# InterDigitalInc/VersatileFilmGrain

Hardware: NVIDIA B200
Metric: 4k_10bit_420_frames_per_sec_device_resident (higher is better)
Workload: dtype int32

## Files before the change

### versatilefilmgrain_b200/csrc/fgs_fast.h

```cpp
#pragma once
#include <stddef.h>
#include <type_traits>
#include "fgs_task.h"

namespace vfgs {

VFGS_HD uint32_t prmt(uint32_t a, uint32_t b, uint32_t sel)
{
#if defined(__CUDA_ARCH__)
	uint32_t d;
	asm("prmt.b32 %0, %1, %2, %3;" : "=r"(d) : "r"(a), "r"(b), "r"(sel));
	return d;
#else
	const uint64_t src = ((uint64_t)b << 32) | a;
	uint32_t d = 0;
	for (int i = 0; i < 4; i++) {
		const uint32_t n = (sel >> (4 * i)) & 0xf;
		uint32_t byte = (uint32_t)(src >> (8 * (n & 7))) & 0xff;
		if (n & 8) byte = (byte & 0x80) ? 0xff : 0x00;
		d |= byte << (8 * i);
	}
	return d;
#endif
}
// ... 651 lines not shown
	g[6] = blend<6>(g[6], u0, u1, w_cur, w_up); g[7] = blend<7>(g[7], u0, u1, w_cur, w_up);
}
template <bool IN16, bool OUT8, int NSH, bool MSB = false>
VFGS_HD void wide_line(const WideLane& L, int rc, int w_cur, int w_up, const WideUp& U, int ru,
                       const uint32_t* raw, uint32_t* outw)
{
	uint32_t a0, a1, b0, b1;
	octet(L.own0 + rc, a0, a1);
	octet(L.own1 + rc, b0, b1);
	int ga[8], gb[8];
	octet_to_ints(a0, a1, ga);
	octet_to_ints(b0, b1, gb);
	int hl = L.has_left ? lds_s8(L.lh + rc) : 0;
	int hr = L.has_right ? lds_s8(L.rh + rc) : 0;
	if (w_cur) {
		uint32_t u0, u1;
		octet(U.own0 + ru, u0, u1);
		blend_octet(ga, u0, u1, w_cur, w_up);
		octet(U.own1 + ru, u0, u1);
		blend_octet(gb, u0, u1, w_cur, w_up);
		if (L.has_left) hl = (hl * w_cur + lds_s8(U.lh + ru) * w_up + 16) >> 5;
		if (L.has_right) hr = (hr * w_cur + lds_s8(U.rh + ru) * w_up + 16) >> 5;
	}
	const int f0 = (hl + 3 * ga[0] + ga[1] + 2) >> 2;
	const int f15 = (gb[6] + 3 * gb[7] + hr + 2) >> 2;
	if (NSH == 3) {
		const int f7 = (ga[6] + 3 * ga[7] + gb[0] + 2) >> 2;
		const int f8 = (ga[7] + 3 * gb[0] + gb[1] + 2) >> 2;
		ga[7] = f7; gb[0] = f8;
	}
	ga[0] = L.has_left ? f0 : ga[0];
	gb[7] = L.has_right ? f15 : gb[7];
	if (IN16) {
		uint32_t cv[8];
		if (MSB) msb_to_lsb<8>(raw, cv);
		const uint32_t* r = MSB ? cv : raw;
		scale_add_clip_16bit<OUT8>(L.lut, L.lo2, L.hi2, ga, r, outw);
		scale_add_clip_16bit<OUT8>(L.lut, L.lo2, L.hi2, gb, r + 4, outw + (OUT8 ? 2 : 4));
	} else {
		scale_add_clip_8bit(L.lut, L.lo2, L.hi2, ga, raw[0], raw[1], outw[0], outw[1]);
		scale_add_clip_8bit(L.lut, L.lo2, L.hi2, gb, raw[2], raw[3], outw[2], outw[3]);
	}
}

#ifndef VFGS_WIDE16_LB
#define VFGS_WIDE16_LB 2
#endif
#ifndef VFGS_WIDE16_LBW
#define VFGS_WIDE16_LBW 4
#endif
#ifndef VFGS_WIDE16_LB8
#define VFGS_WIDE16_LB8 2
#endif
template <bool IN16, bool OUT8, int NSH, bool ALLWIDE = false, bool MSB = false>
VFGS_HD void wide_task_body(const FgsParams& p, smem_addr_t lut, const TaskGeom& t, int k0, int lane)
{
	const int c = t.c;
	const smem_addr_t img = lut + (smem_addr_t)(ptrdiff_t)p.fimg_off[c];
	const Plane& pl = p.comp[c];
	const int ysh = (c && p.suby > 1) ? 1 : 0;
	constexpr int n = 1 << NSH;
	constexpr int LB = !IN16 ? VFGS_FAST_LB16 : OUT8 ? VFGS_WIDE16_LB8 : ALLWIDE ? VFGS_WIDE16_LBW : VFGS_WIDE16_LB;
	static_assert(LB >= 2, "both vertical-overlap lines of a block-row must fall into the first group of lines");
	constexpr int IB = IN16 ? 2 : 1, OB = (IN16 && !OUT8) ? 2 : 1;
	constexpr int RW = IN16 ? 8 : 4, OW = OB == 2 ? 8 : 4;

	const int cl0 = (t.r * 16) >> ysh;
	int cl1 = cl0 + (16 >> ysh);
	if (cl1 > pl.lines) cl1 = pl.lines;
	const int nl = cl1 - cl0;
	if (nl <= 0) return;

	const long long in_pitch = pl.in_row_bytes, out_pitch = pl.out_row_bytes;
	const uint8_t* src = pl.in + (long long)t.f * p.in_frame_bytes + (long long)cl0 * in_pitch + (long long)k0 * IB;
	uint8_t* dst = pl.out + (long long)t.f * p.out_frame_bytes + (long long)cl0 * out_pitch + (long long)k0 * OB;

	uint32_t raw[LB][RW];
#pragma unroll
	for (int q = 0; q < LB; q++) {
		if (IN16) ld_global_32(src + (q < nl ? q : nl - 1) * in_pitch, raw[q]);
		else ld_global_16(src + (q < nl ? q : nl - 1) * in_pitch, raw[q]);
	}

	const int b0 = k0 >> NSH, b1 = (k0 + 15) >> NSH;
	WideLane L;
	L.has_left = b0 > 0;
	L.has_right = b1 + 1 < p.nb;
	L.stride = p.fpat_stride[c];
	L.lut = lut + (smem_addr_t)(c * kLutBytes + lane * 4);
	constexpr int kOutBias = (IN16 && OUT8) ? 2 : 0;
	L.lo2 = (uint32_t)(p.lo[c] + kOutBias) * 0x00010001u; L.hi2 = (uint32_t)(p.hi[c] + kOutBias) * 0x00010001u;

	const int srow = t.r - p.stream_row0;
	const uint16_t* w_cur = p.woffs + (((long long)t.f * p.stream_rows + srow) * p.spitch + 1 + b0) * 4 + c;
	auto windows = [&](const uint16_t* w, smem_addr_t& own0, smem_addr_t& own1, smem_addr_t& lh, smem_addr_t& rh) {
		own0 = img + (smem_addr_t)w[0];
		own1 = NSH == 4 ? own0 + 8 : img + (smem_addr_t)w[4];
		lh = rh = own0;
		if (L.has_left) lh = img + (smem_addr_t)(w[-4] + n - 1);
		if (L.has_right) rh = img + (smem_addr_t)w[NSH == 4 ? 4 : 8];
	};
	windows(w_cur, L.own0, L.own1, L.lh, L.rh);
	WideUp U;
	U.own0 = U.own1 = U.lh = U.rh = L.own0;
	bool ovl = t.r > 0;
	if (ovl) windows(w_cur - p.spitch * 4, U.own0, U.own1, U.lh, U.rh);

	int rc = 0;
	const uint8_t* nxt = src + LB * in_pitch;
#pragma unroll 1
	for (int base = 0; base < nl; base += LB) {
#pragma unroll
		for (int q = 0; q < LB; q++) {
			const int line = base + q;
			uint32_t w[OW];
			int wc = 0, wu = 0, ru = 0;
			if (q == 0 && ovl) { wc = ysh ? 20 : 12; wu = ysh ? 20 : 24; ru = (16 >> ysh) * L.stride; }
			if (q == 1 && ovl && !ysh) { wc = 24; wu = 12; ru = 17 * L.stride; }
			wide_line<IN16, OUT8, NSH, MSB>(L, rc, wc, wu, U, ru, raw[q], w);
			if (MSB && OB == 2) lsb_to_msb<OW>(w);
			if (IN16) ld_global_32_if(nxt, raw[q], line + LB < nl);
			else ld_global_16_if(nxt, raw[q], line + LB < nl);
			if (line < nl) {
				if (OB == 2) st_global_32(dst, w);
				else st_global_16(dst, w);
			}
			rc += L.stride; nxt += in_pitch; dst += out_pitch;
		}
		ovl = false;
	}
}

template <bool OUT8>
VFGS_HD void scale_add_clip_uv_16bit(smem_addr_t lut_u, smem_addr_t lut_v, uint32_t lo2, uint32_t hi2, const int* gu, const int* gv,
                                     const uint32_t raw[4], uint32_t* outw)
{
	constexpr int kRound = OUT8 ? 0x28000 : 0x8000;
	uint32_t r[4];
#pragma unroll
	for (int k = 0; k < 4; k++) {
		const int s_lo = (int)lds32(lut_u | (smem_addr_t)((raw[k] << 5) & 0x7f80u));
		const int s_hi = (int)lds32(lut_v | (smem_addr_t)(shr_fma<11>(raw[k]) & 0x7f80u));
		const int a_lo = s_lo * gu[k] + kRound;
		const int a_hi = s_hi * gv[k] + kRound;
		const uint32_t d2 = prmt((uint32_t)a_lo, (uint32_t)a_hi, 0x7632);
		const uint32_t v2 = min_u16x2(raw[k], 0x3fff3fffu);
		r[k] = min_s16x2(add_max_s16x2(v2, d2, lo2), hi2);
	}
	if (OUT8) {
#pragma unroll
		for (int k = 0; k < 4; k++) r[k] *= 64u;
		outw[0] = prmt(r[0], r[1], 0x7531);
		outw[1] = prmt(r[2], r[3], 0x7531);
	} else {
		outw[0] = r[0]; outw[1] = r[1]; outw[2] = r[2]; outw[3] = r[3];
	}
}
VFGS_HD void scale_add_clip_uv_8bit(smem_addr_t lut_u, smem_addr_t lut_v, uint32_t lo2, uint32_t hi2, const int* gu, const int* gv,
                                    uint32_t raw0, uint32_t raw1, uint32_t& out0, uint32_t& out1)
{
	uint32_t r[4];
#pragma unroll
	for (int k = 0; k < 4; k++) {
		const uint32_t v2 = prmt(k < 2 ? raw0 : raw1, 0u, (k & 1) ? 0x4342 : 0x4140);
		const int s_lo = (int)lds32(lut_u | (smem_addr_t)((v2 << 7) & 0x7f80u));
		const int s_hi = (int)lds32(lut_v | (smem_addr_t)(shr_fma<9>(v2) & 0x7f80u));
		const int a_lo = s_lo * gu[k] + 0x8000;
		const int a_hi = s_hi * gv[k] + 0x8000;
		const uint32_t d2 = prmt((uint32_t)a_lo, (uint32_t)a_hi, 0x7632);
		r[k] = min_s16x2(add_max_s16x2(v2, d2, lo2), hi2);
	}
	out0 = prmt(r[0], r[1], 0x6420);
	out1 = prmt(r[2], r[3], 0x6420);
}

struct UvLane {
	smem_addr_t own_u, own_v;
	smem_addr_t lh_u, rh_u, lh_v, rh_v;
	smem_addr_t lut_u, lut_v;
	int stride;
	bool has_left, has_right;
	uint32_t lo2, hi2;
};
struct UvUp {
	smem_addr_t own_u, own_v, lh_u, rh_u, lh_v, rh_v;
};

VFGS_HD void block_octet(smem_addr_t own, smem_addr_t lh, smem_addr_t rh, smem_addr_t up_own, smem_addr_t up_lh, smem_addr_t up_rh,
                         bool has_left, bool has_right, int rc, int w_cur, int w_up, int ru, int g[8])
{
	uint32_t a0, a1;
	octet(own + rc, a0, a1);
	octet_to_ints(a0, a1, g);
	int hl = has_left ? lds_s8(lh + rc) : 0;
	int hr = has_right ? lds_s8(rh + rc) : 0;
	if (w_cur) {
		uint32_t u0, u1;
		octet(up_own + ru, u0, u1);
		blend_octet(g, u0, u1, w_cur, w_up);
		if (has_left) hl = (hl * w_cur + lds_s8(up_lh + ru) * w_up + 16) >> 5;
		if (has_right) hr = (hr * w_cur + lds_s8(up_rh + ru) * w_up + 16) >> 5;
	}
	const int f0 = (hl + 3 * g[0] + g[1] + 2) >> 2;
	const int f7 = (g[6] + 3 * g[7] + hr + 2) >> 2;
	g[0] = has_left ? f0 : g[0];
	g[7] = has_right ? f7 : g[7];
}

template <bool IN16, bool OUT8>
VFGS_HD void uv_line(const UvLane& L, int rc, int w_cur, int w_up, const UvUp& U, int ru, const uint32_t* raw, uint32_t* outw)
{
	int gu[8], gv[8];
	block_octet(L.own_u, L.lh_u, L.rh_u, U.own_u, U.lh_u, U.rh_u, L.has_left, L.has_right, rc, w_cur, w_up, ru, gu);
	block_octet(L.own_v, L.lh_v, L.rh_v, U.own_v, U.lh_v, U.rh_v, L.has_left, L.has_right, rc, w_cur, w_up, ru, gv);
	if (IN16) {
		uint32_t cv[8];
		msb_to_lsb<8>(raw, cv);
		scale_add_clip_uv_16bit<OUT8>(L.lut_u, L.lut_v, L.lo2, L.hi2, gu, gv, cv, outw);
		scale_add_clip_uv_16bit<OUT8>(L.lut_u, L.lut_v, L.lo2, L.hi2, gu + 4, gv + 4, cv + 4, outw + (OUT8 ? 2 : 4));
	} else {
		scale_add_clip_uv_8bit(L.lut_u, L.lut_v, L.lo2, L.hi2, gu, gv, raw[0], raw[1], outw[0], outw[1]);
		scale_add_clip_uv_8bit(L.lut_u, L.lut_v, L.lo2, L.hi2, gu + 4, gv + 4, raw[2], raw[3], outw[2], outw[3]);
	}
}

template <bool IN16, bool OUT8, bool ALLWIDE = false>
VFGS_HD void uv_task_body(const FgsParams& p, smem_addr_t lut, const TaskGeom& t, int k0, int lane)
{
	const Plane& pl = p.comp[1];
	const int ysh = p.suby > 1 ? 1 : 0;
	constexpr int LB = !IN16 ? VFGS_FAST_LB16 : OUT8 ? VFGS_WIDE16_LB8 : ALLWIDE ? VFGS_WIDE16_LBW : VFGS_WIDE16_LB;
	static_assert(LB >= 2, "both vertical-overlap lines of a block-row must fall into the first group of lines");
	constexpr int IB = IN16 ? 2 : 1, OB = (IN16 && !OUT8) ? 2 : 1;
	constexpr int RW = IN16 ? 8 : 4, OW = OB == 2 ? 8 : 4;

	const int cl0 = (t.r * 16) >> ysh;
	int cl1 = cl0 + (16 >> ysh);
	if (cl1 > pl.lines) cl1 = pl.lines;
	const int nl = cl1 - cl0;
	if (nl <= 0) return;

	const long long in_pitch = pl.in_row_bytes, out_pitch = pl.out_row_bytes;
	const uint8_t* src = pl.in + (long long)t.f * p.in_frame_bytes + (long long)cl0 * in_pitch + (long long)k0 * 2 * IB;
	uint8_t* dst = pl.out + (long long)t.f * p.out_frame_bytes + (long long)cl0 * out_pitch + (long long)k0 * 2 * OB;

	uint32_t raw[LB][RW];
#pragma unroll
	for (int q = 0; q < LB; q++) {
		if (IN16) ld_global_32(src + (q < nl ? q : nl - 1) * in_pitch, raw[q]);
		else ld_global_16(src + (q < nl ? q : nl - 1) * in_pitch, raw[q]);
	}

	const int b = k0 >> 3;
	UvLane L;
	L.has_left = b > 0;
	L.has_right = b + 1 < p.nb;
	L.stride = p.fpat_stride[1];
	L.lut_u = lut + (smem_addr_t)(kLutBytes + lane * 4);
	L.lut_v = lut + (smem_addr_t)(2 * kLutBytes + lane * 4);
	constexpr int kOutBias = (IN16 && OUT8) ? 2 : 0;
	L.lo2 = (uint32_t)(p.lo[1] + kOutBias) * 0x00010001u; L.hi2 = (uint32_t)(p.hi[1] + kOutBias) * 0x00010001u;

	const smem_addr_t img_u = lut + (smem_addr_t)(ptrdiff_t)p.fimg_off[1], img_v = lut + (smem_addr_t)(ptrdiff_t)p.fimg_off[2];
	const int srow = t.r - p.stream_row0;
	const uint16_t* w_u = p.woffs + (((long long)t.f * p.stream_rows + srow) * p.spitch + 1 + b) * 4 + 1;
	auto windows = [&](const uint16_t* w, UvUp& o) {
		o.own_u = img_u + (smem_addr_t)w[0];
		o.own_v = img_v + (smem_addr_t)w[1];
		o.lh_u = o.rh_u = o.own_u; o.lh_v = o.rh_v = o.own_v;
		if (L.has_left) { o.lh_u = img_u + (smem_addr_t)(w[-4] + 7); o.lh_v = img_v + (smem_addr_t)(w[-3] + 7); }
		if (L.has_right) { o.rh_u = img_u + (smem_addr_t)w[4]; o.rh_v = img_v + (smem_addr_t)w[5]; }
	};
	UvUp C;
	windows(w_u, C);
	L.own_u = C.own_u; L.own_v = C.own_v; L.lh_u = C.lh_u; L.rh_u = C.rh_u; L.lh_v = C.lh_v; L.rh_v = C.rh_v;
	UvUp U = C;
	bool ovl = t.r > 0;
	if (ovl) windows(w_u - p.spitch * 4, U);

	int rc = 0;
	const uint8_t* nxt = src + LB * in_pitch;
#pragma unroll 1
	for (int base = 0; base < nl; base += LB) {
#pragma unroll
		for (int q = 0; q < LB; q++) {
			const int line = base + q;
			uint32_t w[OW];
			int wc = 0, wu = 0, ru = 0;
			if (q == 0 && ovl) { wc = ysh ? 20 : 12; wu = ysh ? 20 : 24; ru = (16 >> ysh) * L.stride; }
			if (q == 1 && ovl && !ysh) { wc = 24; wu = 12; ru = 17 * L.stride; }
			uv_line<IN16, OUT8>(L, rc, wc, wu, U, ru, raw[q], w);
			if (OB == 2) lsb_to_msb<OW>(w);
			if (IN16) ld_global_32_if(nxt, raw[q], line + LB < nl);
			else ld_global_16_if(nxt, raw[q], line + LB < nl);
			if (line < nl) {
				if (OB == 2) st_global_32(dst, w);
				else st_global_16(dst, w);
			}
			rc += L.stride; nxt += in_pitch; dst += out_pitch;
		}
		ovl = false;
	}
}

template <bool IN16, bool OUT8, bool EDGE = false, bool ALLWIDE = false, bool SEMI = false>
VFGS_HD void process_task_fast(const FgsParams& p, smem_addr_t lut, uint32_t task, int lane)
{
	TaskGeom t;
	t.f = (int)fastdiv(task, p.div_ftasks);
	uint32_t q = task - (uint32_t)t.f * (uint32_t)p.ftasks_per_frame;
	t.c = 0;
	if (q >= (uint32_t)p.ftasks[0]) { q -= (uint32_t)p.ftasks[0]; t.c = 1; }
	if (t.c == 1 && q >= (uint32_t)p.ftasks[1]) { q -= (uint32_t)p.ftasks[1]; t.c = 2; }
	const uint32_t unit = q * 32u + (uint32_t)lane;
	const uint32_t upr = (uint32_t)p.funits_per_row[t.c];
	if (unit >= upr * (uint32_t)p.rows) return;
	const uint32_t row = fastdiv(unit, p.div_funits[t.c]);
	t.r = p.row_begin + (int)row;
	t.seg = 0;
	static_assert(!(ALLWIDE && EDGE), "the EDGE variant has no wide path");
	static_assert(!(SEMI && EDGE), "the EDGE variant has no semi-planar form");
	if constexpr (SEMI) {
		const int u = (int)(unit - row * upr);
		if (t.c) uv_task_body<IN16, OUT8, ALLWIDE>(p, lut, t, u * 8, lane);
		else wide_task_body<IN16, OUT8, 4, ALLWIDE, IN16>(p, lut, t, u * 16, lane);
		return;
	}
	if (ALLWIDE || (!EDGE && p.fwide[t.c])) {
		const int k0 = (int)(unit - row * upr) * 16;
		if (t.c && p.subx > 1) wide_task_body<IN16, OUT8, 3, ALLWIDE>(p, lut, t, k0, lane);
		else wide_task_body<IN16, OUT8, 4, ALLWIDE>(p, lut, t, k0, lane);
		return;
	}
	if (ALLWIDE) return;
	const int k0 = (int)(unit - row * upr) * kSamplesPerLane;
	if (t.c && p.subx > 1) fast_task_body<IN16, OUT8, 3, EDGE>(p, lut, t, k0, lane);
	else fast_task_body<IN16, OUT8, 4, EDGE>(p, lut, t, k0, lane);
}

}
```

### versatilefilmgrain_b200/csrc/vfgs_b200.cu

```cuda
#include <cuda_runtime.h>
#include <stdarg.h>
#include <stdio.h>
#include <stdlib.h>
#include <string.h>
#include <time.h>
#include <algorithm>
#include <memory>
#include <mutex>
#include <thread>
#include <vector>

#include "../../include/vfgs_b200.h"
#include "../../include/vfgs_fw.h"
#include "../../include/vfgs_hw.h"
#include "../../include/yuv.h"
#include "vfgs_kernels.cuh"
#include "fw_host.h"

using namespace vfgs;

namespace {

struct Slot {
	uint8_t* d_in = nullptr;
// ... 293 lines not shown
}
int make_geometry(Geometry& g, int width, int height, int out_depth) { return make_geometry(g, hw(), width, height, out_depth); }

void fill_common(FgsParams& p, const Geometry& g, const StateRef& s)
{
	memset(&p, 0, sizeof(p));
	fill_state_params(p, *s.h, *s.bi);
	p.nb = g.nb; p.R = g.R;
	p.in_bytes = (int)g.in_sample; p.out_bytes = (int)g.out_sample;
	p.blob = s.img ? s.img->d_blob : nullptr;
	p.fblob = s.img ? s.img->d_fblob : nullptr;
	p.spitch = g.spitch;
}

typedef void (*GrainKernel)(const FgsParams);
enum KernelKind { kGeneral = 0, kFast = 1, kGather = 2, kFastEdge = 3 };

template <bool FOLD, bool SHIFT>
GrainKernel gather_kernel(const FgsParams& p)
{
	if (p.msb_in)
		return p.out_bytes == 1 ? fgs_apply_gather_kernel<true, true, FOLD, SHIFT, true> : fgs_apply_gather_kernel<true, false, FOLD, SHIFT, true>;
	return p.in_bytes == 1 ? fgs_apply_gather_kernel<false, false, FOLD, SHIFT>
	     : p.out_bytes == 1 ? fgs_apply_gather_kernel<true, true, FOLD, SHIFT> : fgs_apply_gather_kernel<true, false, FOLD, SHIFT>;
}
GrainKernel gather_kernel(const FgsParams& p, bool fold, bool shift)
{
	return fold ? (shift ? gather_kernel<true, true>(p) : gather_kernel<true, false>(p))
	            : (shift ? gather_kernel<false, true>(p) : gather_kernel<false, false>(p));
}

int launch_apply(const FgsParams& p, cudaStream_t stream, KernelKind kind = kGeneral, int gather_smem = 0, bool gather_fold = false,
                 bool gather_shift = false)
{
	Context& c = g_ctx;
	if (p.total_tasks <= 0) return VFGS_B200_OK;
	if (p.total_tasks >= (1ll << 31)) return set_err(VFGS_B200_ERR_ARG, "batch too large for one launch (%lld warp-tasks): split the call", p.total_tasks);
	GrainKernel kern = fgs_apply_kernel;
	int threads = kCtaThreads, smem = p.blob_bytes;
	if (kind == kFast || kind == kFastEdge) {
		const bool allwide = kind == kFast && p.in_bytes == 2 && p.out_bytes == 2 && p.fallwide;
		if (kind == kFast && p.ilv[1])
			kern = allwide ? fgs_apply_fast_kernel<true, false, false, true, true>
			     : p.in_bytes == 1 ? fgs_apply_fast_kernel<false, false, false, false, true>
			     : p.out_bytes == 1 ? fgs_apply_fast_kernel<true, true, false, false, true> : fgs_apply_fast_kernel<true, false, false, false, true>;
		else if (allwide)
			kern = fgs_apply_fast_kernel<true, false, false, true>;
		else if (kind == kFast)
			kern = p.in_bytes == 1 ? fgs_apply_fast_kernel<false, false>
			     : p.out_bytes == 1 ? fgs_apply_fast_kernel<true, true> : fgs_apply_fast_kernel<true, false>;
		else
			kern = p.in_bytes == 1 ? fgs_apply_fast_kernel<false, false, true>
			     : p.out_bytes == 1 ? fgs_apply_fast_kernel<true, true, true> : fgs_apply_fast_kernel<true, false, true>;
		threads = fast_threads(p.in_bytes == 2, p.in_bytes == 2 && p.out_bytes == 1, kind == kFastEdge, allwide); smem = p.fsmem;
		if (smem > c.fast_smem_attr) {
			CUDA_TRY(cudaFuncSetAttribute(fgs_apply_fast_kernel<true, false>, cudaFuncAttributeMaxDynamicSharedMemorySize, smem));
			CUDA_TRY(cudaFuncSetAttribute(fgs_apply_fast_kernel<true, true>, cudaFuncAttributeMaxDynamicSharedMemorySize, smem));
			CUDA_TRY(cudaFuncSetAttribute(fgs_apply_fast_kernel<false, false>, cudaFuncAttributeMaxDynamicSharedMemorySize, smem));
			CUDA_TRY(cudaFuncSetAttribute(fgs_apply_fast_kernel<true, false, true>, cudaFuncAttributeMaxDynamicSharedMemorySize, smem));
			CUDA_TRY(cudaFuncSetAttribute(fgs_apply_fast_kernel<true, true, true>, cudaFuncAttributeMaxDynamicSharedMemorySize, smem));
			CUDA_TRY(cudaFuncSetAttribute(fgs_apply_fast_kernel<false, false, true>, cudaFuncAttributeMaxDynamicSharedMemorySize, smem));
			CUDA_TRY(cudaFuncSetAttribute(fgs_apply_fast_kernel<true, false, false, true>, cudaFuncAttributeMaxDynamicSharedMemorySize, smem));
			CUDA_TRY(cudaFuncSetAttribute(fgs_apply_fast_kernel<false, false, false, false, true>, cudaFuncAttributeMaxDynamicSharedMemorySize, smem));
			CUDA_TRY(cudaFuncSetAttribute(fgs_apply_fast_kernel<true, true, false, false, true>, cudaFuncAttributeMaxDynamicSharedMemorySize, smem));
			CUDA_TRY(cudaFuncSetAttribute(fgs_apply_fast_kernel<true, false, false, false, true>, cudaFuncAttributeMaxDynamicSharedMemorySize, smem));
			CUDA_TRY(cudaFuncSetAttribute(fgs_apply_fast_kernel<true, false, false, true, true>, cudaFuncAttributeMaxDynamicSharedMemorySize, smem));
			c.fast_smem_attr = smem;
		}
	} else if (kind == kGather) {
		kern = gather_kernel(p, gather_fold, gather_shift);
		threads = kGatherThreads; smem = gather_smem;
		if (smem > c.gather_smem_attr) {
			FgsParams v = p;
			for (int io = 0; io < 5; io++) {
				v.in_bytes = io == 0 ? 1 : 2; v.out_bytes = io == 2 || io == 4 ? 2 : 1;
				v.msb_in = io >= 3 ? 6 : 0;
				for (int fs = 0; fs < 4; fs++)
					CUDA_TRY(cudaFuncSetAttribute(gather_kernel(v, (fs & 1) != 0, (fs & 2) != 0), cudaFuncAttributeMaxDynamicSharedMemorySize, smem));
			}
			c.gather_smem_attr = smem;
		}
	}
	const int wpc = threads / 32;
	int per_sm = 0;
	CUDA_TRY(cudaOccupancyMaxActiveBlocksPerMultiprocessor(&per_sm, kern, threads, (size_t)smem));
	if (per_sm < 1) return set_err(VFGS_B200_ERR_CUDA, "grain kernel does not fit on an SM (smem %d)", smem);
	long long want = (p.total_tasks + wpc - 1) / wpc;
	long long cap = (long long)c.sm_count * per_sm;
	int grid = (int)(want < cap ? want : cap);
	cudaEvent_t e0 = nullptr, e1 = nullptr;
	if (c.timing) {
		if (c.ev_used == c.ev_begin.size()) {
			cudaEvent_t a, b;
			CUDA_TRY(cudaEventCreate(&a));
			CUDA_TRY(cudaEventCreate(&b));
			c.ev_begin.push_back(a); c.ev_end.push_back(b);
		}
		e0 = c.ev_begin[c.ev_used]; e1 = c.ev_end[c.ev_used]; c.ev_used++;
		CUDA_TRY(cudaEventRecord(e0, stream));
	}
	kern<<<grid, threads, (size_t)smem, stream>>>(p);
	CUDA_TRY(cudaGetLastError());
	if (c.timing) CUDA_TRY(cudaEventRecord(e1, stream));
	g_launches++;
	c.last_launch[0] = grid; c.last_launch[1] = threads; c.last_launch[2] = smem; c.last_launch[3] = c.sm_count;
	c.last_launch[4] |= kind == kFast ? 1 : kind == kGather ? 4 : kind == kFastEdge ? 8 : 2;
	return VFGS_B200_OK;
// ... 1074 lines not shown
```

### versatilefilmgrain_b200/csrc/vfgs_kernels.cuh

```cuda
#pragma once
#include <cuda_runtime.h>
#include "vfgs_tables.h"
#include "fw_device.h"

namespace vfgs {

constexpr int kCtaThreads = 256;
constexpr int kLfsrThreads = 128;
constexpr int kWarpsPerCta = kCtaThreads / 32;

__device__ __forceinline__ uint32_t smem_u32(const void* p)
{
	return (uint32_t)__cvta_generic_to_shared(p);
}
__device__ __forceinline__ void mbar_init(uint64_t* bar, uint32_t count)
{
	asm volatile("mbarrier.init.shared::cta.b64 [%0], %1;" :: "r"(smem_u32(bar)), "r"(count) : "memory");
	asm volatile("fence.mbarrier_init.release.cluster;" ::: "memory");
}
__device__ __forceinline__ void mbar_arrive_expect_tx(uint64_t* bar, uint32_t bytes)
{
	asm volatile("mbarrier.arrive.expect_tx.shared::cta.b64 _, [%0], %1;" :: "r"(smem_u32(bar)), "r"(bytes) : "memory");
}
__device__ __forceinline__ void mbar_wait(uint64_t* bar, uint32_t parity)
// ... 55 lines not shown
                   int nframes, int R, int nb, int spitch, unsigned long long frame0)
{
	const int warp = (int)((blockIdx.x * (unsigned)blockDim.x + threadIdx.x) >> 5);
	const int lane = threadIdx.x & 31;
	if (warp >= nframes * R) return;
	lfsr_row_tables(epoch_state, pow2, states, woffs, wp, warp, R, nb, spitch, frame0, lane);
}

__global__ void __launch_bounds__(kLfsrThreads)
lfsr_states_jobs_kernel(const uint32_t* __restrict__ pow2, const StreamJob* __restrict__ jobs, int njobs, long long nwarps)
{
	const long long warp = (long long)((blockIdx.x * (unsigned long long)blockDim.x + threadIdx.x) >> 5);
	const int lane = threadIdx.x & 31;
	if (warp >= nwarps) return;
	const StreamJob& J = jobs[stream_job_of(jobs, njobs, warp)];
	lfsr_row_tables(J.epoch, pow2, J.states, J.woffs, J.wp, (int)(warp - J.warp0), J.R, J.nb, J.spitch, 0ull, lane);
}

#ifndef VFGS_GENERAL_CTAS
#define VFGS_GENERAL_CTAS 2
#endif
__global__ void __launch_bounds__(kCtaThreads, VFGS_GENERAL_CTAS)
fgs_apply_kernel(const __grid_constant__ FgsParams p)
{
	extern __shared__ __align__(128) uint8_t tab[];
	__shared__ __align__(8) uint64_t bar;

	if (threadIdx.x == 0) mbar_init(&bar, 1);
	__syncthreads();
	if (threadIdx.x == 0) {
		mbar_arrive_expect_tx(&bar, (uint32_t)p.blob_bytes);
		bulk_copy_g2s(tab, p.blob, (uint32_t)p.blob_bytes, &bar);
	}
	mbar_wait(&bar, 0);

	const int lane = threadIdx.x & 31;
	const long long stride = (long long)gridDim.x * kWarpsPerCta;
	for (long long task = (long long)blockIdx.x * kWarpsPerCta + (threadIdx.x >> 5); task < p.total_tasks; task += stride)
		process_task(p, tab, (uint32_t)task, lane);
}

#ifndef VFGS_FAST_THREADS8
#define VFGS_FAST_THREADS8 768
#endif
#ifndef VFGS_FAST_THREADS16
#define VFGS_FAST_THREADS16 768
#endif
#ifndef VFGS_FAST_THREADS_IN8
#define VFGS_FAST_THREADS_IN8 896
#endif
#ifndef VFGS_FAST_THREADS_EDGE
#define VFGS_FAST_THREADS_EDGE 768
#endif
#ifndef VFGS_FAST_THREADS16W
#define VFGS_FAST_THREADS16W 512
#endif
template <bool IN16, bool OUT8, bool EDGE = false, bool ALLWIDE = false> struct FastCta {
	static_assert(!ALLWIDE || (IN16 && !OUT8 && !EDGE), "ALLWIDE exists for 16-bit input and output only");
	static constexpr int threads = ALLWIDE ? VFGS_FAST_THREADS16W : EDGE ? VFGS_FAST_THREADS_EDGE : !IN16 ? VFGS_FAST_THREADS_IN8 : OUT8 ? VFGS_FAST_THREADS8 : VFGS_FAST_THREADS16;
};
inline int fast_threads(bool in16, bool out8, bool edge = false, bool allwide = false)
{
	return allwide ? VFGS_FAST_THREADS16W : edge ? VFGS_FAST_THREADS_EDGE : !in16 ? VFGS_FAST_THREADS_IN8 : out8 ? VFGS_FAST_THREADS8 : VFGS_FAST_THREADS16;
}

template <bool IN16, bool OUT8, bool EDGE = false, bool ALLWIDE = false, bool SEMI = false>
__global__ void __launch_bounds__(FastCta<IN16, OUT8, EDGE, ALLWIDE>::threads, 1)
fgs_apply_fast_kernel(const __grid_constant__ FgsParams p)
{
	constexpr int kFastThreads = FastCta<IN16, OUT8, EDGE, ALLWIDE>::threads, kFastWarps = kFastThreads / 32;
	extern __shared__ __align__(128) uint8_t smem[];
	__shared__ __align__(8) uint64_t bar;

	const uint32_t pad = (0u - smem_u32(smem)) & (uint32_t)(kLutAlign - 1);
	if (p.probe) {
		if (threadIdx.x == 0) *p.probe = pad;
		return;
	}
#ifdef VFGS_DEBUG_ASSERTS
	if (pad != (uint32_t)p.fpad) __trap();
#endif
	uint8_t* lut_ptr = smem + pad;

	if (threadIdx.x == 0) mbar_init(&bar, 1);
	__syncthreads();
	if (threadIdx.x == 0) {
		mbar_arrive_expect_tx(&bar, (uint32_t)(p.fimg_bytes[0] + p.fimg_bytes[1] + p.fimg_bytes[2]));
		for (int c = 0; c < 3; c++)
			if (p.fimg_bytes[c]) bulk_copy_g2s(lut_ptr + p.fimg_off[c], p.fblob + p.fimg_src[c], (uint32_t)p.fimg_bytes[c], &bar);
	}
	expand_fast_luts((uint32_t*)lut_ptr, (const uint32_t*)p.fblob, (uint32_t)p.pow16, threadIdx.x, kFastThreads);
	mbar_wait(&bar, 0);
	__syncthreads();

	const int lane = threadIdx.x & 31;
	const smem_addr_t lut = smem_addr(lut_ptr);
	const long long stride = (long long)gridDim.x * kFastWarps;
	for (long long task = (long long)blockIdx.x * kFastWarps + (threadIdx.x >> 5); task < p.total_tasks; task += stride)
		process_task_fast<IN16, OUT8, EDGE, ALLWIDE, SEMI>(p, lut, (uint32_t)task, lane);
}

__device__ __forceinline__ void multi_switch_barrier()
{
	__syncthreads();
	if (threadIdx.x == 0) asm volatile("fence.proxy.async.shared::cta;" ::: "memory");
}

template <bool IN16, bool OUT8, bool EDGE = false, bool ALLWIDE = false, bool SEMI = false>
__global__ void __launch_bounds__(FastCta<IN16, OUT8, EDGE, ALLWIDE>::threads, 1)
fgs_apply_fast_multi_kernel(const __grid_constant__ MultiParams m)
{
	constexpr int kFastThreads = FastCta<IN16, OUT8, EDGE, ALLWIDE>::threads, kFastWarps = kFastThreads / 32;
	extern __shared__ __align__(128) uint8_t smem[];
	__shared__ __align__(8) uint64_t bar;

	const uint32_t pad = (0u - smem_u32(smem)) & (uint32_t)(kLutAlign - 1);
	if (m.probe) {
		if (threadIdx.x == 0) *m.probe = pad;
		return;
	}
	uint8_t* lut_ptr = smem + pad;
	if (threadIdx.x == 0) mbar_init(&bar, 1);
	__syncthreads();

	const int lane = threadIdx.x & 31, warp = threadIdx.x >> 5;
	const smem_addr_t lut = smem_addr(lut_ptr);
	MultiCursor cur;
	multi_begin(m.task0, m.njobs, (int)gridDim.x, (int)blockIdx.x, cur);
	uint32_t phase = 0;
	int j;
	long long lo, end;
	while (multi_next(m.task0, cur, j, lo, end)) {
		const long long t0 = m.task0[j];
		const FgsParams& p = m.jobs[j];
		if (phase) multi_switch_barrier();
		if (threadIdx.x == 0) {
			mbar_arrive_expect_tx(&bar, (uint32_t)(p.fimg_bytes[0] + p.fimg_bytes[1] + p.fimg_bytes[2]));
			for (int c = 0; c < 3; c++)
				if (p.fimg_bytes[c]) bulk_copy_g2s(lut_ptr + p.fimg_off[c], p.fblob + p.fimg_src[c], (uint32_t)p.fimg_bytes[c], &bar);
		}
		expand_fast_luts((uint32_t*)lut_ptr, (const uint32_t*)p.fblob, (uint32_t)p.pow16, threadIdx.x, kFastThreads);
		mbar_wait(&bar, phase & 1);
		phase++;
		__syncthreads();
		for (long long task = lo + warp; task < end; task += kFastWarps)
			process_task_fast<IN16, OUT8, EDGE, ALLWIDE, SEMI>(p, lut, (uint32_t)(task - t0), lane);
	}
}

#ifndef VFGS_GATHER_THREADS
#define VFGS_GATHER_THREADS 896
#define VFGS_GATHER_CTAS 1
// ... 114 lines not shown
```

### versatilefilmgrain_b200/csrc/vfgs_tables.h

```cpp
#pragma once
#include <stdint.h>
#include <string.h>
#include <vector>

#include "fgs_gather.h"

#ifndef VFGS_PAT_ROW_SKEW
#define VFGS_PAT_ROW_SKEW 8
#endif
#ifndef VFGS_FAST_WIDE8
#define VFGS_FAST_WIDE8 1
#endif
#ifndef VFGS_FAST_WIDE16
#define VFGS_FAST_WIDE16 1
#endif
#ifndef VFGS_FAST_ROW_SKEW
#define VFGS_FAST_ROW_SKEW 8
#endif

namespace vfgs {

constexpr int kSlots = 9;

struct HwState {
// ... 256 lines not shown
	for (int which = 0; which < 2; which++) {
		const int k = which ? 3 : 0;
		FgsParams& f = which ? lp.edge : lp.fast;
		bool served[3];
		for (int c = 0; c < 3; c++) served[c] = kind[c] == k;
		place_fast_images(f, bi, fast_pad, served);
		if (f.fsmem + 64 > smem_limit) {
			for (int c = 0; c < 3; c++) if (kind[c] == k) { kind[c] = 2; served[c] = false; }
			place_fast_images(f, bi, fast_pad, served);
		}
	}
	lp.gather_fold = ngather > 0;
	for (int c = 0; c < 3; c++) if (kind[c] == 1 && !bi.neg_ok[c ? 1 : 0]) lp.gather_fold = false;
	if (lp.gather_fold && kLutAlign + ngather * kLutBytes + bi.gbytes > smem_limit) lp.gather_fold = false;
#ifdef VFGS_GATHER_NO_FOLD
	lp.gather_fold = false;
#endif
	lp.gather_smem = kLutAlign + ngather * kLutBytes + (lp.gather_fold ? bi.gbytes : bi.bytes);
	if (ngather && lp.gather_smem > smem_limit) {
		for (int c = 0; c < 3; c++) if (kind[c] == 1) kind[c] = 2;
		ngather = 0; lp.gather_fold = false;
	}
	int gi = 0;
	for (int c = 0; c < 3; c++) {
		lp.gather.glut_index[c] = kind[c] == 1 ? gi++ : -1;
		if (kind[c] != 0) lp.fast.nseg[c] = 0;
		if (kind[c] != 1) lp.gather.nseg[c] = 0;
		if (kind[c] != 2) lp.general.nseg[c] = 0;
		if (kind[c] != 3) lp.edge.nseg[c] = 0;
		(kind[c] == 0 ? lp.any_fast : kind[c] == 1 ? lp.any_gather : kind[c] == 3 ? lp.any_edge : lp.any_general) = true;
	}
	for (int which = 0; which < 2; which++) {
		const int k = which ? 3 : 0;
		FgsParams& f = which ? lp.edge : lp.fast;
		f.ftasks_per_frame = 0;
		for (int c = 0; c < 3; c++) {
			const bool wide_on = f.in_bytes == 1 ? VFGS_FAST_WIDE8 != 0 : VFGS_FAST_WIDE16 != 0;
			f.fwide[c] = wide_on && kind[c] == 0 && k == 0 && f.comp[c].width % 16 == 0 &&
			             aligned_for(f.comp[c].in, f.comp[c].in_row_bytes, f.in_frame_bytes, (size_t)(16 * f.in_bytes)) &&
			             aligned_for(f.comp[c].out, f.comp[c].out_row_bytes, f.out_frame_bytes, (size_t)(16 * f.out_bytes));
			f.funits_per_row[c] = kind[c] == k ? (f.comp[c].width + (f.fwide[c] ? 16 : kSamplesPerLane) - 1) / (f.fwide[c] ? 16 : kSamplesPerLane) : 0;
			if (semi && c) {
				f.fwide[c] = c == 1 && kind[1] == k;
				f.funits_per_row[c] = f.fwide[c] ? f.comp[1].width / 8 : 0;
			}
			f.ftasks[c] = (f.funits_per_row[c] * f.rows + 31) / 32;
			f.ftasks_per_frame += f.ftasks[c];
			f.div_funits[c] = make_fastdiv((uint32_t)(f.funits_per_row[c] > 0 ? f.funits_per_row[c] : 1));
		}
		f.div_ftasks = make_fastdiv((uint32_t)(f.ftasks_per_frame > 0 ? f.ftasks_per_frame : 1));
		int served = 0, wide = 0;
		for (int c = 0; c < (semi ? 2 : 3); c++) if (kind[c] == k) { served++; wide += f.fwide[c] ? 1 : 0; }
		f.fallwide = served > 0 && wide == served;
	}
	lp.gather_shift = in_place && ngather > 0;
	lp.gather.ngather = ngather;
	lp.gather.gpat_off[0] = bi.pat_off[0]; lp.gather.gpat_off[1] = bi.pat_off[1];
	lp.gather.gneg_off[0] = bi.neg_off[0]; lp.gather.gneg_off[1] = bi.neg_off[1];
	lp.gather.gslot_mul[0] = (uint32_t)bi.pat_size[0]; lp.gather.gslot_mul[1] = (uint32_t)bi.pat_size[1];
	lp.gather.blob_bytes = lp.gather_fold ? bi.gbytes : bi.bytes;
	{
		FgsParams& g = lp.gather;
		g.gtasks_per_frame = 0;
		for (int c = 0; c < 3; c++) {
			const bool block8 = c && g.subx > 1;
			const int upr = kind[c] == 1 ? ((g.comp[c].width + kSamplesPerLane - 1) / kSamplesPerLane + 1) & ~1 : 0;
			const long long units = (long long)upr * g.rows;
			g.gunits_per_row[c] = upr;
			(void)block8;
			g.gtasks[c] = kind[c] != 1 ? 0 : (int)((units + (lp.gather_shift ? 1 : 0) + 31) / 32);
			g.gtasks_per_frame += g.gtasks[c];
			g.div_gunits[c] = make_fastdiv((uint32_t)(upr > 0 ? upr : 1));
		}
		g.div_gtasks = make_fastdiv((uint32_t)(g.gtasks_per_frame > 0 ? g.gtasks_per_frame : 1));
	}
	for (FgsParams* q : {&lp.fast, &lp.gather, &lp.general, &lp.edge}) {
		q->tasks_per_stripe = q->nseg[0] + q->nseg[1] + q->nseg[2];
		q->total_tasks = (long long)q->nframes * q->rows * q->tasks_per_stripe;
		q->div_tps = make_fastdiv((uint32_t)(q->tasks_per_stripe > 0 ? q->tasks_per_stripe : 1));
	}
	lp.fast.total_tasks = (long long)lp.fast.nframes * lp.fast.ftasks_per_frame;
	lp.edge.total_tasks = (long long)lp.edge.nframes * lp.edge.ftasks_per_frame;
	lp.gather.total_tasks = (long long)lp.gather.nframes * lp.gather.gtasks_per_frame;
}

inline bool in_place_needs_scratch(const LaunchPlan& lp, const TableInfo& bi)
{
	for (int c = 0; c < 3; c++)
		if (lp.kind[c] == 2 && bi.uniform_pi[c] < 0) return true;
	return false;
}

struct WoffParams {
	WoffComp c[3];
};
inline WoffParams make_woff_params(const FgsParams& p, const int kind[3])
{
	WoffParams w;
	for (int c = 0; c < 3; c++) {
		const int stepx = (c && p.subx > 1) ? 2 : 4, stepy = (c && p.suby > 1) ? 2 : 4;
		WoffComp& k = w.c[c];
		if (kind[c] == 1) {
			k.off0 = 0; k.doff = 0x8000; k.ystride = stepy * p.pat_stride[c ? 1 : 0];
			k.copy = 0; k.kmask = 0; k.kshift = 0; k.xmul = stepx;
		} else {
			k.off0 = p.fpat_off[c][0]; k.doff = p.fpat_off[c][1] - p.fpat_off[c][0]; k.ystride = stepy * p.fpat_stride[c];
// ... 116 lines not shown
```

Measured before the change: 128,400.

## Prefetch input lines through a per-warp cp.async shared-memory ring in ALLWIDE kernel

For the 16-bit all-wide fast path, each lane now streams its input lines through a per-warp ring of cp.async slots in shared memory. Prefetching runs across task boundaries, so the next task's first lines are already in flight while the current one finishes, replacing the register prefetch that restarted each task. The cost is extra shared memory per CTA, which may disable the all-wide variant when it does not fit. It also adds cp.async wait and shared-load overhead on every line.

```diff
diff --git a/versatilefilmgrain_b200/csrc/fgs_fast.h b/versatilefilmgrain_b200/csrc/fgs_fast.h
--- a/versatilefilmgrain_b200/csrc/fgs_fast.h
+++ b/versatilefilmgrain_b200/csrc/fgs_fast.h
@@ -727,8 +727,122 @@
 #ifndef VFGS_WIDE16_LB8
 #define VFGS_WIDE16_LB8 2
 #endif
-template <bool IN16, bool OUT8, int NSH, bool ALLWIDE = false, bool MSB = false>
-VFGS_HD void wide_task_body(const FgsParams& p, smem_addr_t lut, const TaskGeom& t, int k0, int lane)
+
+VFGS_HD bool fast_task_lane(const FgsParams& p, uint32_t task, int lane, TaskGeom& t, int& u)
+{
+	t.f = (int)fastdiv(task, p.div_ftasks);
+	uint32_t q = task - (uint32_t)t.f * (uint32_t)p.ftasks_per_frame;
+	t.c = 0;
+	if (q >= (uint32_t)p.ftasks[0]) { q -= (uint32_t)p.ftasks[0]; t.c = 1; }
+	if (t.c == 1 && q >= (uint32_t)p.ftasks[1]) { q -= (uint32_t)p.ftasks[1]; t.c = 2; }
+	const uint32_t unit = q * 32u + (uint32_t)lane;
+	const uint32_t upr = (uint32_t)p.funits_per_row[t.c];
+	if (unit >= upr * (uint32_t)p.rows) return false;
+	const uint32_t row = fastdiv(unit, p.div_funits[t.c]);
+	t.r = p.row_begin + (int)row;
+	t.seg = 0;
+	u = (int)(unit - row * upr);
+	return true;
+}
+
+#ifndef VFGS_FAST_THREADS16W
+#define VFGS_FAST_THREADS16W 512
+#endif
+#ifndef VFGS_WIDE16_RING
+#define VFGS_WIDE16_RING 4
+#endif
+constexpr int kRingSlots = VFGS_WIDE16_RING;
+constexpr int kRingSlotBytes = 32 * 32;
+constexpr int kRingLB = VFGS_WIDE16_LBW;
+VFGS_HD int wide_ring_offset(int fsmem) { return (fsmem + 127) & ~127; }
+VFGS_HD int wide_ring_smem(int fsmem, int warps) { return wide_ring_offset(fsmem) + warps * kRingSlots * kRingSlotBytes; }
+
+struct LineRing {
+	smem_addr_t base;
+	int slot;
+	uint32_t task, stride;
+	int left, valid;
+	const uint8_t* src;
+	long long pitch;
+};
+
+VFGS_HD void cp_async_32(smem_addr_t dst, const uint8_t* src)
+{
+#if defined(__CUDA_ARCH__)
+	asm volatile("cp.async.cg.shared.global [%0], [%1], 16;\n\tcp.async.cg.shared.global [%2], [%3], 16;"
+	             :: "r"(dst), "l"(src), "r"(dst + 16), "l"(src + 16) : "memory");
+#else
+	memcpy((void*)dst, src, 32);
+#endif
+}
+VFGS_HD void cp_async_commit()
+{
+#if defined(__CUDA_ARCH__)
+	asm volatile("cp.async.commit_group;" ::: "memory");
+#endif
+}
+template <int N>
+VFGS_HD void cp_async_wait()
+{
+#if defined(__CUDA_ARCH__)
+	asm volatile("cp.async.wait_group %0;" :: "n"(N) : "memory");
+#endif
+}
+VFGS_HD void lds256(smem_addr_t a, uint32_t r[8])
+{
+#if defined(__CUDA_ARCH__)
+	asm volatile("ld.shared.v4.u32 {%0,%1,%2,%3}, [%8];\n\tld.shared.v4.u32 {%4,%5,%6,%7}, [%8+16];"
+	             : "=r"(r[0]), "=r"(r[1]), "=r"(r[2]), "=r"(r[3]), "=r"(r[4]), "=r"(r[5]), "=r"(r[6]), "=r"(r[7]) : "r"(a) : "memory");
+#else
+	memcpy(r, (const void*)a, 32);
+#endif
+}
+
+VFGS_HD void ring_request(LineRing& R, const FgsParams& p, int lane)
+{
+	while (R.left == 0) {
+		if ((long long)R.task >= p.total_tasks) { R.left = 1 << 30; R.valid = 0; break; }
+		TaskGeom t;
+		int u;
+		if (fast_task_lane(p, R.task, lane, t, u)) {
+			const Plane& pl = p.comp[t.c];
+			const int ysh = (t.c && p.suby > 1) ? 1 : 0;
+			const int cl0 = (t.r * 16) >> ysh;
+			int cl1 = cl0 + (16 >> ysh);
+			if (cl1 > pl.lines) cl1 = pl.lines;
+			const int nl = cl1 - cl0;
+			if (nl > 0) {
+				R.valid = nl;
+				R.left = (nl + kRingLB - 1) / kRingLB * kRingLB;
+				R.pitch = pl.in_row_bytes;
+				R.src = pl.in + (long long)t.f * p.in_frame_bytes + (long long)cl0 * R.pitch + (long long)u * 32;
+			}
+		}
+		R.task += R.stride;
+	}
+	if (R.valid > 0) cp_async_32(R.base + (smem_addr_t)(R.slot * kRingSlotBytes), R.src);
+	cp_async_commit();
+	R.src += R.pitch; R.left--; R.valid--;
+}
+VFGS_HD void ring_begin(LineRing& R, const FgsParams& p, smem_addr_t base, uint32_t task, uint32_t stride, int lane)
+{
+	R.base = base; R.task = task; R.stride = stride; R.left = 0; R.valid = 0; R.src = nullptr; R.pitch = 0;
+	for (R.slot = 0; R.slot < kRingSlots; R.slot++) ring_request(R, p, lane);
+	R.slot = 0;
+}
+VFGS_HD void ring_line(LineRing& R, uint32_t raw[8])
+{
+	cp_async_wait<kRingSlots - 1>();
+	lds256(R.base + (smem_addr_t)(R.slot * kRingSlotBytes), raw);
+}
+VFGS_HD void ring_refill(LineRing& R, const FgsParams& p, int lane)
+{
+	ring_request(R, p, lane);
+	R.slot = R.slot + 1 == kRingSlots ? 0 : R.slot + 1;
+}
+
+template <bool IN16, bool OUT8, int NSH, bool ALLWIDE = false, bool MSB = false, bool RING = false>
+VFGS_HD void wide_task_body(const FgsParams& p, smem_addr_t lut, const TaskGeom& t, int k0, int lane, LineRing* ring = nullptr)
 {
 	const int c = t.c;
 	const smem_addr_t img = lut + (smem_addr_t)(ptrdiff_t)p.fimg_off[c];
@@ -750,11 +864,14 @@
 	const uint8_t* src = pl.in + (long long)t.f * p.in_frame_bytes + (long long)cl0 * in_pitch + (long long)k0 * IB;
 	uint8_t* dst = pl.out + (long long)t.f * p.out_frame_bytes + (long long)cl0 * out_pitch + (long long)k0 * OB;
 
+	static_assert(!RING || (IN16 && RW == 8 && LB == kRingLB), "the line ring holds 32-byte lines of 16-bit samples, kRingLB per group");
 	uint32_t raw[LB][RW];
-#pragma unroll
-	for (int q = 0; q < LB; q++) {
-		if (IN16) ld_global_32(src + (q < nl ? q : nl - 1) * in_pitch, raw[q]);
-		else ld_global_16(src + (q < nl ? q : nl - 1) * in_pitch, raw[q]);
+	if constexpr (!RING) {
+#pragma unroll
+		for (int q = 0; q < LB; q++) {
+			if (IN16) ld_global_32(src + (q < nl ? q : nl - 1) * in_pitch, raw[q]);
+			else ld_global_16(src + (q < nl ? q : nl - 1) * in_pitch, raw[q]);
+		}
 	}
 
 	const int b0 = k0 >> NSH, b1 = (k0 + 15) >> NSH;
@@ -792,9 +909,11 @@
 			int wc = 0, wu = 0, ru = 0;
 			if (q == 0 && ovl) { wc = ysh ? 20 : 12; wu = ysh ? 20 : 24; ru = (16 >> ysh) * L.stride; }
 			if (q == 1 && ovl && !ysh) { wc = 24; wu = 12; ru = 17 * L.stride; }
+			if constexpr (RING) ring_line(*ring, raw[q]);
 			wide_line<IN16, OUT8, NSH, MSB>(L, rc, wc, wu, U, ru, raw[q], w);
 			if (MSB && OB == 2) lsb_to_msb<OW>(w);
-			if (IN16) ld_global_32_if(nxt, raw[q], line + LB < nl);
+			if constexpr (RING) ring_refill(*ring, p, lane);
+			else if (IN16) ld_global_32_if(nxt, raw[q], line + LB < nl);
 			else ld_global_16_if(nxt, raw[q], line + LB < nl);
 			if (line < nl) {
 				if (OB == 2) st_global_32(dst, w);
@@ -899,8 +1018,8 @@
 	}
 }
 
-template <bool IN16, bool OUT8, bool ALLWIDE = false>
-VFGS_HD void uv_task_body(const FgsParams& p, smem_addr_t lut, const TaskGeom& t, int k0, int lane)
+template <bool IN16, bool OUT8, bool ALLWIDE = false, bool RING = false>
+VFGS_HD void uv_task_body(const FgsParams& p, smem_addr_t lut, const TaskGeom& t, int k0, int lane, LineRing* ring = nullptr)
 {
 	const Plane& pl = p.comp[1];
 	const int ysh = p.suby > 1 ? 1 : 0;
@@ -919,11 +1038,14 @@
 	const uint8_t* src = pl.in + (long long)t.f * p.in_frame_bytes + (long long)cl0 * in_pitch + (long long)k0 * 2 * IB;
 	uint8_t* dst = pl.out + (long long)t.f * p.out_frame_bytes + (long long)cl0 * out_pitch + (long long)k0 * 2 * OB;
 
+	static_assert(!RING || (IN16 && RW == 8 && LB == kRingLB), "the line ring holds 32-byte lines of 16-bit samples, kRingLB per group");
 	uint32_t raw[LB][RW];
-#pragma unroll
-	for (int q = 0; q < LB; q++) {
-		if (IN16) ld_global_32(src + (q < nl ? q : nl - 1) * in_pitch, raw[q]);
-		else ld_global_16(src + (q < nl ? q : nl - 1) * in_pitch, raw[q]);
+	if constexpr (!RING) {
+#pragma unroll
+		for (int q = 0; q < LB; q++) {
+			if (IN16) ld_global_32(src + (q < nl ? q : nl - 1) * in_pitch, raw[q]);
+			else ld_global_16(src + (q < nl ? q : nl - 1) * in_pitch, raw[q]);
+		}
 	}
 
 	const int b = k0 >> 3;
@@ -964,9 +1086,11 @@
 			int wc = 0, wu = 0, ru = 0;
 			if (q == 0 && ovl) { wc = ysh ? 20 : 12; wu = ysh ? 20 : 24; ru = (16 >> ysh) * L.stride; }
 			if (q == 1 && ovl && !ysh) { wc = 24; wu = 12; ru = 17 * L.stride; }
+			if constexpr (RING) ring_line(*ring, raw[q]);
 			uv_line<IN16, OUT8>(L, rc, wc, wu, U, ru, raw[q], w);
 			if (OB == 2) lsb_to_msb<OW>(w);
-			if (IN16) ld_global_32_if(nxt, raw[q], line + LB < nl);
+			if constexpr (RING) ring_refill(*ring, p, lane);
+			else if (IN16) ld_global_32_if(nxt, raw[q], line + LB < nl);
 			else ld_global_16_if(nxt, raw[q], line + LB < nl);
 			if (line < nl) {
 				if (OB == 2) st_global_32(dst, w);
@@ -978,8 +1102,8 @@
 	}
 }
 
-template <bool IN16, bool OUT8, bool EDGE = false, bool ALLWIDE = false, bool SEMI = false>
-VFGS_HD void process_task_fast(const FgsParams& p, smem_addr_t lut, uint32_t task, int lane)
+template <bool IN16, bool OUT8, bool EDGE = false, bool ALLWIDE = false, bool SEMI = false, bool RING = false>
+VFGS_HD void process_task_fast(const FgsParams& p, smem_addr_t lut, uint32_t task, int lane, LineRing* ring = nullptr)
 {
 	TaskGeom t;
 	t.f = (int)fastdiv(task, p.div_ftasks);
@@ -995,16 +1119,17 @@
 	t.seg = 0;
 	static_assert(!(ALLWIDE && EDGE), "the EDGE variant has no wide path");
 	static_assert(!(SEMI && EDGE), "the EDGE variant has no semi-planar form");
+	static_assert(!RING || ALLWIDE, "only the ALLWIDE variant has a line ring");
 	if constexpr (SEMI) {
 		const int u = (int)(unit - row * upr);
-		if (t.c) uv_task_body<IN16, OUT8, ALLWIDE>(p, lut, t, u * 8, lane);
-		else wide_task_body<IN16, OUT8, 4, ALLWIDE, IN16>(p, lut, t, u * 16, lane);
+		if (t.c) uv_task_body<IN16, OUT8, ALLWIDE, RING>(p, lut, t, u * 8, lane, ring);
+		else wide_task_body<IN16, OUT8, 4, ALLWIDE, IN16, RING>(p, lut, t, u * 16, lane, ring);
 		return;
 	}
 	if (ALLWIDE || (!EDGE && p.fwide[t.c])) {
 		const int k0 = (int)(unit - row * upr) * 16;
-		if (t.c && p.subx > 1) wide_task_body<IN16, OUT8, 3, ALLWIDE>(p, lut, t, k0, lane);
-		else wide_task_body<IN16, OUT8, 4, ALLWIDE>(p, lut, t, k0, lane);
+		if (t.c && p.subx > 1) wide_task_body<IN16, OUT8, 3, ALLWIDE, false, RING>(p, lut, t, k0, lane, ring);
+		else wide_task_body<IN16, OUT8, 4, ALLWIDE, false, RING>(p, lut, t, k0, lane, ring);
 		return;
 	}
 	if (ALLWIDE) return;
diff --git a/versatilefilmgrain_b200/csrc/vfgs_b200.cu b/versatilefilmgrain_b200/csrc/vfgs_b200.cu
--- a/versatilefilmgrain_b200/csrc/vfgs_b200.cu
+++ b/versatilefilmgrain_b200/csrc/vfgs_b200.cu
@@ -369,7 +369,8 @@
 		else
 			kern = p.in_bytes == 1 ? fgs_apply_fast_kernel<false, false, true>
 			     : p.out_bytes == 1 ? fgs_apply_fast_kernel<true, true, true> : fgs_apply_fast_kernel<true, false, true>;
-		threads = fast_threads(p.in_bytes == 2, p.in_bytes == 2 && p.out_bytes == 1, kind == kFastEdge, allwide); smem = p.fsmem;
+		threads = fast_threads(p.in_bytes == 2, p.in_bytes == 2 && p.out_bytes == 1, kind == kFastEdge, allwide);
+		smem = allwide ? wide_ring_smem(p.fsmem, threads / 32) : p.fsmem;
 		if (smem > c.fast_smem_attr) {
 			CUDA_TRY(cudaFuncSetAttribute(fgs_apply_fast_kernel<true, false>, cudaFuncAttributeMaxDynamicSharedMemorySize, smem));
 			CUDA_TRY(cudaFuncSetAttribute(fgs_apply_fast_kernel<true, true>, cudaFuncAttributeMaxDynamicSharedMemorySize, smem));
diff --git a/versatilefilmgrain_b200/csrc/vfgs_kernels.cuh b/versatilefilmgrain_b200/csrc/vfgs_kernels.cuh
--- a/versatilefilmgrain_b200/csrc/vfgs_kernels.cuh
+++ b/versatilefilmgrain_b200/csrc/vfgs_kernels.cuh
@@ -131,9 +131,6 @@
 #ifndef VFGS_FAST_THREADS_EDGE
 #define VFGS_FAST_THREADS_EDGE 768
 #endif
-#ifndef VFGS_FAST_THREADS16W
-#define VFGS_FAST_THREADS16W 512
-#endif
 template <bool IN16, bool OUT8, bool EDGE = false, bool ALLWIDE = false> struct FastCta {
 	static_assert(!ALLWIDE || (IN16 && !OUT8 && !EDGE), "ALLWIDE exists for 16-bit input and output only");
 	static constexpr int threads = ALLWIDE ? VFGS_FAST_THREADS16W : EDGE ? VFGS_FAST_THREADS_EDGE : !IN16 ? VFGS_FAST_THREADS_IN8 : OUT8 ? VFGS_FAST_THREADS8 : VFGS_FAST_THREADS16;
@@ -175,8 +172,18 @@
 	const int lane = threadIdx.x & 31;
 	const smem_addr_t lut = smem_addr(lut_ptr);
 	const long long stride = (long long)gridDim.x * kFastWarps;
-	for (long long task = (long long)blockIdx.x * kFastWarps + (threadIdx.x >> 5); task < p.total_tasks; task += stride)
-		process_task_fast<IN16, OUT8, EDGE, ALLWIDE, SEMI>(p, lut, (uint32_t)task, lane);
+	const long long first = (long long)blockIdx.x * kFastWarps + (threadIdx.x >> 5);
+	if constexpr (ALLWIDE) {
+		LineRing ring;
+		ring_begin(ring, p, smem_addr(smem) + (smem_addr_t)(wide_ring_offset(p.fsmem) + (threadIdx.x >> 5) * kRingSlots * kRingSlotBytes + lane * 32),
+		           (uint32_t)first, (uint32_t)stride, lane);
+		for (long long task = first; task < p.total_tasks; task += stride)
+			process_task_fast<IN16, OUT8, EDGE, ALLWIDE, SEMI, true>(p, lut, (uint32_t)task, lane, &ring);
+		cp_async_wait<0>();
+	} else {
+		for (long long task = first; task < p.total_tasks; task += stride)
+			process_task_fast<IN16, OUT8, EDGE, ALLWIDE, SEMI>(p, lut, (uint32_t)task, lane);
+	}
 }
 
 __device__ __forceinline__ void multi_switch_barrier()
diff --git a/versatilefilmgrain_b200/csrc/vfgs_tables.h b/versatilefilmgrain_b200/csrc/vfgs_tables.h
--- a/versatilefilmgrain_b200/csrc/vfgs_tables.h
+++ b/versatilefilmgrain_b200/csrc/vfgs_tables.h
@@ -332,6 +332,8 @@
 		int served = 0, wide = 0;
 		for (int c = 0; c < (semi ? 2 : 3); c++) if (kind[c] == k) { served++; wide += f.fwide[c] ? 1 : 0; }
 		f.fallwide = served > 0 && wide == served;
+		if (f.fallwide && f.in_bytes == 2 && f.out_bytes == 2 && wide_ring_smem(f.fsmem, VFGS_FAST_THREADS16W / 32) + 64 > smem_limit)
+			f.fallwide = false;
 	}
 	lp.gather_shift = in_place && ngather > 0;
 	lp.gather.ngather = ngather;
```

Result: slower. 117,700, median of 6 (-8.4%).
